# EspressoSystems/cap

Hardware: AMD Instinct MI355X
Metric: transfer-note proofs/sec (2-in/2-out) (higher is better)
Workload: dtype u32 limbs (254-bit Montgomery integers; 9 x 29-bit lazy limbs in the hot kernels)

## Files before the change

cap_amd/csrc/curve29.hpp:

```cpp
#pragma once
#include "curve.hpp"
#include "field29.hpp"

namespace cap {

struct g1a {
  fl x, y;
};
struct g1x {
  fl x, y, zz, zzz;
};

template <int SCHED>
struct G1LT {
  using F = Fl<FqP29, SCHED>;

  static CAP_HD bool all_zero(const fl& a) {
    uint32_t o = 0;
#pragma unroll
    for (int i = 0; i < 9; i++) o |= a.v[i];
    return o == 0;
  }
  static CAP_HD bool is_inf(const g1x& p) { return all_zero(p.zz); }
  static CAP_HD bool is_inf(const g1a& p) { return all_zero(p.x) && all_zero(p.y); }
// ... 116 lines not shown
    const fl p = F::sub(u2, a.x);
    if (F::is_zero(p)) return false;
#if defined(__HIP_DEVICE_COMPILE__)
    asm volatile("; madd_acc: common path");
#endif
    const fl r = F::sub(s2, a.y);
    const fl pp = F::sqr(p);
    const fl ppp = F::mul(p, pp);
    const fl qq = F::mul(a.x, pp);
    g1x o;
    o.x = F::weak_reduce(F::sub_from_lazy(F::sub2p_lazy(F::sqr(r), ppp), F::add(qq, qq)));
    o.y = F::mul_add_mul(r, F::sub2p_lazy(qq, o.x), F::neg4p_lazy(a.y), ppp);
    o.zz = F::mul(a.zz, pp);
    o.zzz = F::mul(a.zzz, ppp);
    a = o;
    return true;
  }
  static CAP_HD bool add_acc(g1x& a, const g1x& b) {
    const fl u1 = F::mul(a.x, b.zz);
    const fl u2 = F::mul(b.x, a.zz);
    const fl p = F::sub(u2, u1);
    if (F::is_zero(p)) return false;
    const fl s1 = F::mul(a.y, b.zzz);
    const fl s2 = F::mul(b.y, a.zzz);
    const fl r = F::sub(s2, s1);
    const fl pp = F::sqr(p);
    const fl ppp = F::mul(p, pp);
    const fl qq = F::mul(u1, pp);
    g1x o;
    o.x = F::weak_reduce(F::sub_from_lazy(F::sub2p_lazy(F::sqr(r), ppp), F::add(qq, qq)));
// ... 102 lines not shown
```

cap_amd/csrc/msm.hip:

```cpp
#define CAP_FL_SCHED 1
#include "msm.hpp"
#include "msm_recode.hpp"
#include "curve29.hpp"
#include "quad29.hpp"
#include "launch.hpp"

#include <math.h>
#include <stdio.h>

#include <atomic>
#include <stdlib.h>

namespace cap {

namespace {

constexpr int kThreads = 256;
constexpr uint32_t kDigitTile = 1024;
constexpr int kDigitThreads = 1024;
constexpr uint32_t kMinItemLen = 32, kMaxItemLen = 512;
constexpr uint32_t kBatchItemCap = 256;

using G1S = G1LT<0>;

// ... 894 lines not shown
      if ((uint64_t)chunk * blockDim.x >= n_items) break;
      it = chunk * blockDim.x + threadIdx.x;
    } else {
      it = (blockIdx.x + round * gridDim.x) * blockDim.x + threadIdx.x;
      if ((uint64_t)(blockIdx.x + round * gridDim.x) * blockDim.x >= n_items) break;
    }
    if (it >= n_items) continue;
  const uint32_t gb = item_bucket[it], j = item_sub[it];
  const uint32_t b = gb / half;
  const uint32_t cnt = counts[gb];
  const uint32_t items = (cnt + item_len - 1) / item_len;
  const uint32_t q = cnt / items, r = cnt - q * items;
  const uint32_t lo = j * q + (j < r ? j : r), hi = lo + q + (j < r ? 1u : 0u);
  const uint32_t* lst = sorted + (size_t)b * per + offsets[gb];
  g1x acc = G1L::inf();
  for (uint32_t e = lo; e < hi; e++) {
    const uint32_t v = lst[e];
    const g1a pt = G1L::load(ext[v & 0x7FFFFFFFu]);
    const bool negate = (v >> 31) != 0;
    if (__builtin_expect(G1L::is_inf(pt) || !G1L::madd_acc(acc, pt, negate), 0)) acc = G1L::add_mixed(acc, pt, negate);
  }
  if (items == 1) buckets[gb] = G1L::store(acc);
  else item_pts[item_base[b] + item_off[gb] + j] = G1L::store(acc);
  }
}

__global__ __launch_bounds__(kThreads) void msm_reduce_segments(const g1_xyzz* __restrict__ buckets, uint32_t half,
                                                                uint32_t seg_len, uint32_t nseg, uint32_t batch,
                                                                g1_xyzz* __restrict__ seg_pts) {
  uint32_t t = blockIdx.x * blockDim.x + threadIdx.x;
  if (t >= nseg * batch) return;
// ... 1701 lines not shown
```

cap_amd/csrc/ntt.hip:

```cpp
#include "ntt.hpp"
#include "field29.hpp"
#include "launch.hpp"

#include <stdlib.h>

#include <vector>

namespace cap {

namespace {

constexpr int kThreads = 256;
#ifndef CAP_NTT_IO_BATCH
#define CAP_NTT_IO_BATCH 2
#endif
constexpr int kIoBatch = CAP_NTT_IO_BATCH;
#ifdef CAP_NTT_WAVES4
#define CAP_NTT_ATTR __attribute__((amdgpu_waves_per_eu(4, 4)))
#else
#define CAP_NTT_ATTR
#endif
constexpr uint32_t kMaxTileLogDefault = 10;
uint32_t max_tile_log() {
  static uint32_t v = [] {
// ... 22 lines not shown
  uint32_t in_group;
  uint32_t in_es;
  size_t in_inner2;
  uint32_t in_group2;
  size_t out_outer, out_inner;
  uint32_t out_group;
  size_t out_inner2;
  uint32_t out_group2;
  size_t pre_inner;
  const fl* tw_small;
  const fe* tw_full;
  const fe* pre_scale;
  const fe* post_scale;
  fe post_scalar;
  uint32_t use_post_scalar;
  uint32_t lazy_out;
  uint32_t log_n;
  uint32_t log_len;
  uint32_t log_c;
  uint32_t log_m;
  uint32_t log_n1, log_n2;
  uint32_t* tile_counter;
  uint32_t tiles_x, tiles_y;
};

__device__ __forceinline__ bool next_tile(const PassParams& p, uint32_t round, uint32_t& bx, uint32_t& by) {
  if (!p.tile_counter) {
    bx = blockIdx.x;
    by = blockIdx.y;
    return round == 0;
// ... 152 lines not shown
      if (p.pre_scale && any[u] && nz) v = Fr29::mul(v, Fr29::load(pre[u]));
      sh[(bitrev32(j, p.log_len) << p.log_c) + c] = v;
    }
  }
  __syncthreads();
  lds_ntt(sh, p.tw_small, p.log_len, p.log_c);
  const uint32_t tw_shift = p.log_n - p.log_m;
  for (uint32_t e0 = threadIdx.x; e0 < tile; e0 += kIoBatch * kThreads) {
    fe tw[kIoBatch];
    size_t exs[kIoBatch];
#pragma unroll
    for (int u = 0; u < kIoBatch; u++) {
      const uint32_t e = e0 + u * kThreads;
      const uint32_t c = e & cmask, k = e >> p.log_c;
      exs[u] = e < tile ? ((size_t)(col0 + c) * k) << tw_shift : 0;
      if (exs[u]) tw[u] = p.tw_full[exs[u]];
    }
#pragma unroll
    for (int u = 0; u < kIoBatch; u++) {
      const uint32_t e = e0 + u * kThreads;
      if (e >= tile) break;
      const uint32_t c = e & cmask, k = e >> p.log_c;
      fl v = sh[e];
      v = exs[u] ? Fr29::mul(v, Fr29::load(tw[u])) : Fr29::weak_reduce(v);
      out[base + ((size_t)k << log_s) + c] = Fr29::pack(v);
    }
  }
  }
}
template <bool PERSIST>
__global__ __launch_bounds__(kThreads) CAP_NTT_ATTR void ntt_col_pass(PassParams p) {
  extern __shared__ __align__(16) unsigned char smem[];
  fl* sh = reinterpret_cast<fl*>(smem);
  if constexpr (!PERSIST) {
    col_tile(p, sh, blockIdx.x, blockIdx.y);
  } else {
    uint32_t bx, by;
    for (uint32_t round = 0; next_tile(p, round, bx, by); round++) col_tile(p, sh, bx, by);
  }
// ... 235 lines not shown
  hipError_t e;
  if ((e = hipMalloc(&d->tw_fwd, sizeof(fe) * n)) != hipSuccess) return (int)e;
  if ((e = hipMalloc(&d->tw_inv, sizeof(fe) * n)) != hipSuccess) return (int)e;
  if ((e = hipMalloc(&d->coset_fwd, sizeof(fe) * n)) != hipSuccess) return (int)e;
  if ((e = hipMalloc(&d->coset_inv, sizeof(fe) * n)) != hipSuccess) return (int)e;
  fe w = host_root_of_unity(log_n);
  fe g = host_from_u64(5);
  d->n_inv = Fr::inv(host_from_u64((uint64_t)n));
  int rc;
  if ((rc = build_powers(d->tw_fwd, n, w, nullptr, stream))) return rc;
  if ((rc = build_powers(d->tw_inv, n, Fr::inv(w), nullptr, stream))) return rc;
  if ((rc = build_powers(d->coset_fwd, n, g, nullptr, stream))) return rc;
  if ((rc = build_powers(d->coset_inv, n, Fr::inv(g), &d->n_inv, stream))) return rc;
  fe* src[4] = {d->tw_fwd, d->tw_inv, d->coset_fwd, d->coset_inv};
  fe** dst[4] = {&d->tw29_fwd, &d->tw29_inv, &d->coset29_fwd, &d->coset29_inv};
  for (int k = 0; k < 4; k++) {
    if ((e = hipMalloc(dst[k], sizeof(fe) * n)) != hipSuccess) return (int)e;
    launch("table_to_internal", table_to_internal, dim3((unsigned)((n + 255) / 256)), dim3(256), 0, stream, *dst[k],
           (const fe*)src[k], n);
  }
  d->n_inv29 = Fr29::pack(Fr29::canonical(Fr29::from_ext(d->n_inv)));
  if ((e = hipStreamSynchronize(stream)) != hipSuccess) return (int)e;
  hipFree(d->tw_inv);
  hipFree(d->coset_fwd);
  hipFree(d->coset_inv);
  d->tw_inv = d->coset_fwd = d->coset_inv = nullptr;
  return 0;
}

void ntt_free_domain(NttDomain* d) {
  if (d->tw_fwd) hipFree(d->tw_fwd);
  if (d->tw_inv) hipFree(d->tw_inv);
  if (d->coset_fwd) hipFree(d->coset_fwd);
  if (d->coset_inv) hipFree(d->coset_inv);
  for (fe* t : {d->tw29_fwd, d->tw29_inv, d->coset29_fwd, d->coset29_inv})
    if (t) hipFree(t);
  d->tw_fwd = d->tw_inv = d->coset_fwd = d->coset_inv = nullptr;
  d->tw29_fwd = d->tw29_inv = d->coset29_fwd = d->coset29_inv = nullptr;
}

void ntt_table_to_internal(fe* out, const fe* in, size_t n, hipStream_t stream) {
  if (n == 0) return;
  launch("table_to_internal", table_to_internal, dim3((unsigned)((n + 255) / 256)), dim3(256), 0, stream, out, in, n);
}

namespace {
unsigned ntt_persistent() {
  static const unsigned v = [] {
    const char* e = getenv("CAPGPU_NTT_PERSISTENT");
    const long x = e ? atol(e) : 0;
    return (unsigned)(x >= 1 && x <= 16 ? x : 0);
  }();
  return v;
// ... 116 lines not shown
  auto set_out = [&](const Addr& a) {
    p.out_outer = a.outer;
    p.out_inner = a.inner;
    p.out_group = a.group;
    p.out_group2 = 1;
    p.out_inner2 = 0;
    if (&a == &a_dst && io && io->dst_group2 > 1) {
      p.out_group2 = io->dst_group2;
      p.out_inner2 = io->dst_inner2;
    }
  };
  p.pre_inner = io ? io->pre_inner : 0;
  p.log_n = log_n;
  p.tw_full = tw_full;
  p.use_post_scalar = 0;

  const fe* pre = (!dir && coset) ? dom.coset29_fwd : nullptr;
  if (io && io->pre_scale) pre = io->pre_scale;
  bool first = true;
  const fe* cur_in = io ? io->src : data;
  uint32_t log_m = log_n;
  for (int d = 0; d < passes - 1; d++) {
    const uint32_t log_len = plan.digits[d], log_c = plan.log_c[d];
    p.in = cur_in;
    p.out = scratch;
    set_in(first ? a_src : a_tmp, first ? src_len : ~(size_t)0, first ? src_es : 1);
    set_out(a_tmp);
    p.tw_small = reinterpret_cast<const fl*>(tws[log_len]);
    p.pre_scale = first ? pre : nullptr;
    p.post_scale = nullptr;
    p.log_len = log_len;
    p.log_c = log_c;
    p.log_m = log_m;
    size_t lds = sizeof(fl) << (log_len + log_c);
    launch_pass("ntt_col_pass", ntt_col_pass<false>, ntt_col_pass<true>, p, small, (size_t)plan.tiles[d], count, lds,
                plan.persistent[d] != 0, stream);
    cur_in = scratch;
    first = false;
    log_m -= log_len;
  }
  {
    const int last = passes - 1;
    const uint32_t log_len = plan.digits[last], log_c = plan.log_c[last];
    const uint32_t log_n1 = passes >= 2 ? plan.digits[0] : 0;
    const uint32_t log_n2 = passes == 3 ? plan.digits[1] : 0;
    p.in = cur_in;
    p.out = data;
    set_in(first ? a_src : a_tmp, first ? src_len : ~(size_t)0, first ? src_es : 1);
    set_out(a_dst);
    p.tw_small = reinterpret_cast<const fl*>(tws[log_len]);
    p.pre_scale = first ? pre : nullptr;
    p.post_scale = (dir && coset) ? dom.coset29_inv : nullptr;
    p.use_post_scalar = (dir && !coset) ? 1 : 0;
    p.post_scalar = (io && io->has_post_scalar) ? io->post_scalar : dom.n_inv29;
    p.lazy_out = (io && io->lazy_out) ? 1 : 0;
    p.log_len = log_len;
    p.log_c = log_c;
    p.log_n1 = log_n1;
    p.log_n2 = log_n2;
    size_t lds = sizeof(fl) << (log_len + log_c);
    launch_pass("ntt_row_pass", ntt_row_pass<false>, ntt_row_pass<true>, p, small, (size_t)plan.tiles[last], count, lds,
                plan.persistent[last] != 0, stream);
  }
  return 0;
}

namespace {
void exponent_third(uint32_t e[8]) {
// ... 114 lines not shown
```

cap_amd/csrc/ntt.hpp:

```cpp
#pragma once
#include <hip/hip_runtime.h>
#include <stdint.h>

#include "field.hpp"

namespace cap {

struct NttDomain {
  uint32_t log_n = 0;
  fe* tw_fwd = nullptr;
  fe* tw_inv = nullptr;
  fe* coset_fwd = nullptr;
  fe* coset_inv = nullptr;
  fe n_inv;
  fe* tw29_fwd = nullptr;
  fe* tw29_inv = nullptr;
  fe* coset29_fwd = nullptr;
  fe* coset29_inv = nullptr;
  fe n_inv29;
};

constexpr int kMaxLogTile = 11;
struct NttSmallTables {
  fe* fwd[kMaxLogTile + 1] = {nullptr};
  fe* inv[kMaxLogTile + 1] = {nullptr};
  uint32_t* fwd_u[kMaxLogTile + 1] = {nullptr};
  uint32_t* inv_u[kMaxLogTile + 1] = {nullptr};
  uint32_t* pass_counters = nullptr;
  mutable uint32_t next_counter = 0;
};
constexpr uint32_t kNttPassCounters = 256;
// ... 61 lines not shown
```

cap_amd/csrc/plonk.hip:

```cpp
#define CAP_FL_SCHED 1
#include <stdlib.h>
#include <string.h>

#include <algorithm>
#include <atomic>
#include <chrono>
#include <condition_variable>
#include <functional>
#include <map>
#include <mutex>
#include <string>
#include <thread>
#include <vector>

#include "check_kernels.hpp"
#include "coalescer.hpp"
#include "context.hpp"
#include "host_util.hpp"
#include "launch.hpp"
#include "params.hpp"
#include "plonk_kernels.hpp"
#include "tickets.hpp"
#include "transcript_dev.hpp"
#include "vars_kernels.hpp"
// ... 529 lines not shown
      x = Fr::mul(x, w6);
    }
  }
  const Ntt3Domain* dom_m = nullptr;
  if ((rc = get_domain3(K.log_m, &dom_m))) return rc;
  launch("k_inv_nx1", k_inv_nx1, dim3(cdiv(m, kThreads)), dim3(kThreads), 0, s, K.inv_nx1, (const fe*)dom_m->xs_ext,
         fr_from_u64((uint64_t)n), m);
  ntt_table_to_internal(K.inv_nx1, K.inv_nx1, m, s);
  {
    auto conv = [](const fe& a) { return Fr29::pack(Fr29::canonical(Fr29::from_ext(a))); };
    K.qc29.g = conv(K.qc.g);
    for (int i = 0; i < NW; i++) K.qc29.k[i] = conv(K.qc.k[i]);
    for (int i = 0; i < 8; i++) K.qc29.zh_inv[i] = conv(K.qc.zh_inv[i]);
  }
  if (!K.recompute) {
    CAP_HIP(hipMalloc(&K.pk_coset, sizeof(fe) * 18 * m));
    if ((rc = compute_pk_coset(s, K, K.pk_coset))) return rc;
  }
  return CAPGPU_OK;
}

void key_set_vk(ProvingKey& K, const std::vector<g1_affine>& ha) {
  memset(&K.vk, 0, sizeof(K.vk));
  K.vk.domain_size = K.n;
  K.vk.num_inputs = K.num_inputs;
  for (int i = 0; i < NW; i++) fe_to_words(K.qc.k[i], K.vk.k[i]);
  for (int i = 0; i < NS; i++) affine_to_words(ha[i], K.vk.selector_comms[i]);
  for (int i = 0; i < NW; i++) affine_to_words(ha[NS + i], K.vk.sigma_comms[i]);
  SolidityTranscript t;
  t.append_u64_le(254);
  t.append_u64_le((uint64_t)K.n);
  t.append_u64_le((uint64_t)K.num_inputs);
// ... 147 lines not shown
  K->qc = src.qc;
  K->qc29 = src.qc29;
  K->vk = src.vk;
  K->vk_bytes = src.vk_bytes;
  K->recompute = src.recompute;
  K->device = c.device;
  auto dup = [&](fe** dst, const fe* from, size_t count) -> int {
    if (!from) return CAPGPU_OK;
    CAP_HIP(hipMalloc(dst, sizeof(fe) * count));
    CAP_HIP(copy_between(*dst, c.device, from, src_device, sizeof(fe) * count, c.stream));
    return CAPGPU_OK;
  };
  int rc;
  if ((rc = dup(&K->coef, src.coef, 18 * src.ps))) return rc;
  if ((rc = dup(&K->sig_eval, src.sig_eval, (size_t)NW * src.n))) return rc;
  if ((rc = dup(&K->pk_coset, src.pk_coset, 18 * src.m))) return rc;
  if ((rc = dup(&K->inv_nx1, src.inv_nx1, src.m))) return rc;
  {
    std::lock_guard<std::mutex> lk(src.chk_mu);
    if (src.wire_vars && src.chk_perm) {
      const size_t bytes = sizeof(uint32_t) * NW * src.n;
      CAP_HIP(hipMalloc(&K->wire_vars, bytes));
      CAP_HIP(hipMalloc(&K->chk_perm, bytes));
      CAP_HIP(copy_between(K->wire_vars, c.device, src.wire_vars, src_device, bytes, c.stream));
      CAP_HIP(copy_between(K->chk_perm, c.device, src.chk_perm, src_device, bytes, c.stream));
      K->num_vars = src.num_vars;
    }
  }
  CAP_HIP(hipStreamSynchronize(c.stream));
  *out = K;
  return CAPGPU_OK;
// ... 1729 lines not shown
```

cap_amd/csrc/plonk_kernels.hpp:

```cpp
#pragma once
#include <hip/hip_runtime.h>

#include "field.hpp"
#include "field29.hpp"

namespace cap {
namespace pk {

constexpr int NW = 5;
constexpr int NS = 13;
constexpr int kThreads = 256;
constexpr int kScanPerThread = 4;
constexpr int kScanBlock = kThreads * kScanPerThread;

struct Chal {
  fe beta, gamma, alpha, alpha2;
};

struct QuotConst {
  fe g;
  fe k[NW];
  fe zh_inv[8];
};

__global__ __launch_bounds__(kThreads) void k_pad_copy(fe* __restrict__ dst, size_t dst_outer, size_t dst_inner,
                                                       const fe* __restrict__ src, size_t src_outer, size_t src_inner,
                                                       uint32_t inner, size_t len, size_t total) {
  size_t k = (size_t)blockIdx.x * blockDim.x + threadIdx.x;
  if (k >= total) return;
  uint32_t q = blockIdx.y;
  size_t d = (size_t)(q / inner) * dst_outer + (size_t)(q % inner) * dst_inner + k;
// ... 185 lines not shown
struct ColAcc {
  uint64_t c[18];
  __device__ __forceinline__ void clear() {
#pragma unroll
    for (int k = 0; k < 18; k++) c[k] = 0;
  }
  __device__ __forceinline__ void mad(const fl& a, const fl& b) {
#pragma unroll
    for (int i = 0; i < 9; i++)
#pragma unroll
      for (int j = 0; j < 9; j++) c[i + j] += (uint64_t)a.v[i] * b.v[j];
  }
  __device__ __forceinline__ fl reduce() { return Fr29::reduce_cols(c); }
};

__global__ __launch_bounds__(kThreads) void k_quotient(const fe* __restrict__ pkc, const fe* const* __restrict__ pkc_of,
                                                       const fe* __restrict__ cos, const fe* __restrict__ xs,
                                                       const fe* __restrict__ inv_nx1,
                                                       const Chal* __restrict__ chal, QuotConst qc, size_t m,
                                                       fe* __restrict__ t_out) {
  using F = Fr29;
  size_t i = (size_t)blockIdx.y * blockDim.x + threadIdx.x;
  if (i >= m) return;
  const uint32_t p = blockIdx.x;
  if (pkc_of) pkc = pkc_of[p];
  const uint32_t mm = (uint32_t)(m / 3);
  const uint32_t blk = (i >= mm ? 1u : 0u) + (i >= 2 * (size_t)mm ? 1u : 0u);
  const fe* c = cos + (size_t)p * 6 * m;
  auto sel = [&](int s) { return F::load(pkc[(size_t)s * m + i]); };
  fl w0 = F::load(c[i]), w1 = F::load(c[m + i]), w2 = F::load(c[2 * m + i]), w3 = F::load(c[3 * m + i]),
     w4 = F::load(c[4 * m + i]);
  fl w01 = F::mul(w0, w1), w23 = F::mul(w2, w3);
  ColAcc acc;
  acc.clear();
  acc.mad(sel(0), w0);
  acc.mad(sel(1), w1);
  acc.mad(sel(2), w2);
  acc.mad(sel(3), w3);
  acc.mad(sel(4), w01);
// ... 2 lines not shown
  acc.clear();
  {
    fl t = F::sqr(w0);
    acc.mad(sel(6), F::mul(F::sqr(t), w0));
    t = F::sqr(w1);
    acc.mad(sel(7), F::mul(F::sqr(t), w1));
    t = F::sqr(w2);
    acc.mad(sel(8), F::mul(F::sqr(t), w2));
    t = F::sqr(w3);
    acc.mad(sel(9), F::mul(F::sqr(t), w3));
  }
  acc.mad(sel(12), F::mul(F::mul(w01, w23), w4));
  acc.mad(F::neg(sel(10)), w4);
  fl gate2 = acc.reduce();
  fl total = F::normalize(F::add(F::add(gate, gate2), sel(11)));
  const fl beta = F::load(chal[p].beta), gamma = F::load(chal[p].gamma);
  const fl zx = F::load(c[5 * m + i]);
  {
    fl x = F::load(xs[i]);
    fl bx = F::mul(beta, x);
    const uint32_t k1 = (uint32_t)i - blk * mm;
    const size_t inext = (size_t)blk * mm + ((k1 + 2) & (mm - 1));
    fl a = zx, b = F::load(c[5 * m + inext]);
    fl wg = F::add(w0, gamma);
    a = F::mul(a, F::normalize(F::add(wg, bx)));
    b = F::mul(b, F::normalize(F::add(wg, F::mul(beta, sel(NS + 0)))));
    wg = F::add(w1, gamma);
    a = F::mul(a, F::normalize(F::add(wg, F::mul(F::load(qc.k[1]), bx))));
    b = F::mul(b, F::normalize(F::add(wg, F::mul(beta, sel(NS + 1)))));
    wg = F::add(w2, gamma);
    a = F::mul(a, F::normalize(F::add(wg, F::mul(F::load(qc.k[2]), bx))));
    b = F::mul(b, F::normalize(F::add(wg, F::mul(beta, sel(NS + 2)))));
    wg = F::add(w3, gamma);
    a = F::mul(a, F::normalize(F::add(wg, F::mul(F::load(qc.k[3]), bx))));
    b = F::mul(b, F::normalize(F::add(wg, F::mul(beta, sel(NS + 3)))));
    wg = F::add(w4, gamma);
    a = F::mul(a, F::normalize(F::add(wg, F::mul(F::load(qc.k[4]), bx))));
// ... 150 lines not shown
```

cap_amd/csrc/prove_run.hpp:

```cpp
#pragma once
#include "context.hpp"
#include "host_util.hpp"
#include "launch.hpp"
#include "params.hpp"
#include "plonk_kernels.hpp"
#include "transcript_dev.hpp"
#include "vars_kernels.hpp"

namespace cap {
namespace {

inline unsigned cdiv(size_t a, size_t b) { return (unsigned)((a + b - 1) / b); }

void pad_copy(hipStream_t s, fe* dst, size_t dst_outer, size_t dst_inner, const fe* src, size_t src_outer,
              size_t src_inner, uint32_t inner, uint32_t count, size_t len, size_t total) {
  if (count == 0 || total == 0) return;
  launch("k_pad_copy", k_pad_copy, dim3(cdiv(total, kThreads), count), dim3(kThreads), 0, s, dst, dst_outer, dst_inner,
         src, src_outer, src_inner, inner, len, total);
}

template <int OP, int REV>
void scan_exclusive(hipStream_t s, const fe* in, fe* out, size_t len, size_t stride, uint32_t batch, fe* tot) {
  uint32_t nblocks = cdiv(len, kScanBlock);
  launch(OP == 0 ? "k_scan_local_mul" : "k_scan_local_add", k_scan_local<OP, REV>, dim3(nblocks, batch), dim3(kThreads),
// ... 133 lines not shown
BatchWs carve(void* base, const ProvingKey& K, uint32_t P, size_t num_inputs, bool coeffs, uint32_t tr_stride = 0) {
  Carver c(base);
  BatchWs w{};
  size_t n = K.n, m = K.m, ps = K.ps;
  w.wpoly = c.take<fe>((size_t)P * NW * ps);
  w.wev = coeffs ? c.take<fe>((size_t)P * NW * n) : nullptr;
  w.pi = num_inputs ? c.take<fe>((size_t)P * n) : nullptr;
  w.num = c.take<fe>((size_t)P * n);
  w.den = c.take<fe>((size_t)P * n);
  w.pre = c.take<fe>((size_t)P * n);
  w.sfx = c.take<fe>((size_t)P * n);
  w.scan_tot = c.take<fe>((size_t)P * 2 * (cdiv(ps, kScanBlock) + 1));
  w.inv_total = c.take<fe>(P);
  w.zpoly = c.take<fe>((size_t)P * ps);
  w.coset = c.take<fe>((size_t)P * 6 * m);
  w.pkc = K.recompute ? c.take<fe>((size_t)18 * m) : nullptr;
  w.t = c.take<fe>((size_t)P * m);
  w.pows = c.take<fe>((size_t)P * 4 * ps);
  w.pw = c.take<fe>((size_t)P * 4 * 24);
  w.pows_small = c.take<fe>((size_t)P * 4 * (kPowLow + (ps + kPowLow - 1) / kPowLow));
  w.batchpoly = c.take<fe>((size_t)P * 2 * ps);
  w.hbuf = c.take<fe>((size_t)P * 2 * ps);
  w.quot = c.take<fe>((size_t)P * 2 * ps);
  w.evals = c.take<fe>((size_t)P * 10);
  w.eval_partial = c.take<fe>((size_t)P * 10 * kEvalChunks);
  w.d_pub = c.take<fe>((size_t)P * (num_inputs ? num_inputs : 1));
  w.d_blind = c.take<fe>((size_t)P * 13);
  w.chal = c.take<Chal>(P);
  w.chal29 = c.take<Chal>(P);
  w.flags = c.take<uint32_t>(P);
  w.comms = c.take<g1_jac>((size_t)P * 5);
// ... 3 lines not shown
  if (tr_stride) {
    w.d_proofs = c.take<uint8_t>((size_t)P * td::kPrBytes);
    w.zeta = c.take<fe>(P);
    w.tr_state = c.take<uint8_t>((size_t)P * 64);
    w.tr_app = c.take<uint8_t>((size_t)P * td::kAppBytes);
    w.tr_pre_len = c.take<uint32_t>(P);
    w.tr_pre = c.take<uint8_t>((size_t)P * tr_stride);
  }
  w.total = c.off + 256;
  return w;
}

int compute_pk_coset(hipStream_t s, const ProvingKey& K, fe* dst) {
  return run_ntt3_fwd(s, K.log_m, dst, 18, NttIo{K.coef, K.ps, 0, K.n, 1, K.m, 0, 1});
}

std::atomic<int> g_wire_commit{-1};
bool wire_commit_from_evals() {
  static const int env_default = [] {
    const char* e = getenv("CAPGPU_WIRE_COMMIT");
    return (e && (!strcmp(e, "coeffs") || !strcmp(e, "0"))) ? 0 : 1;
  }();
  const int m = g_wire_commit.load(std::memory_order_relaxed);
  return (m < 0 ? env_default : m) != 0;
}

std::atomic<int> g_transcript{-1};
int transcript_mode() {
  static const int env_default = [] {
    const char* e = getenv("CAPGPU_TRANSCRIPT");
// ... 160 lines not shown
    if (!sizing) trace("pb_lagrange_fallback", c.slot, rc);
  }
  pl.dev_tr = transcript_mode() == CAPGPU_TRANSCRIPT_DEVICE && !comm_shard_prover();
  if (pl.dev_tr) {
    if (longest_prefix > (1u << 30)) {
      set_error("capgpu_plonk_prove: transcript init message of %zu bytes", longest_prefix);
      return CAPGPU_ERR_INVALID_ARG;
    }
    pl.tr_stride = transcript_stride(longest_prefix);
  }
  pl.inv_on_device = perm_inv_on_device() || pl.dev_tr;
  pl.chunks = pl.r1_copies ? h2d_chunks(P) : 1;
  const bool own = !c.prof.on && c.stream == c.own_stream;
  pl.overlap = pl.chunks == 1 && P <= r1_overlap_max() && (sizing || (own && !comm_shard_prover())) &&
               (pl.s2 = side_stream(c)) != nullptr;
  pl.graphs = P <= graph_max_batch() && pl.chunks == 1 && own && comm_shard_slot() < 0;
  *out = pl;
  return CAPGPU_OK;
}

struct ProveNeeds {
  size_t prove_ws = 0, msm_ws = 0, ntt_scratch = 0, stage_a = 0, stage_b = 0, pinned = 0;
  void ntt(size_t bytes) { ntt_scratch = std::max(ntt_scratch, bytes); }
  void msm(const MsmBases& T, size_t len, uint32_t batch) { msm_ws = std::max(msm_ws, msm_workspace_bytes(T, len, batch)); }
};

struct ProveRequest {
  const fe* d_wires = nullptr;
  const uint64_t* pub_inputs = nullptr;
  size_t num_inputs = 0;
  const uint64_t* blinders = nullptr;
// ... 26 lines not shown
  const uint32_t P;
  const size_t n, m, ps, num_inputs;
  const fe* const d_wires;
  const uint64_t* pub_inputs;
  const uint64_t* const* h_wires;
  const NttDomain* dom_n = nullptr;
  const Ntt3Domain* dom_q = nullptr;
  const fe omega;
  std::vector<uint64_t> pub_rows;
  std::vector<const fe*> key_ptrs;
  const fe* const* sig_of = nullptr;
  const fe* const* pkc_of = nullptr;
  std::vector<SolidityTranscript> tr;
  g1_jac* hj = nullptr;
  fe* h_tot = nullptr;
  fe* h_evals = nullptr;
  uint32_t* h_flags = nullptr;
  uint8_t* h_proofs = nullptr;
  const size_t proofs_bytes;
  std::vector<g1_affine> ha;

  ProveRun(Context& c_, const ProvePlan& pl_, const ProvingKey& K_, const ProveRequest& rq_)
      : side_drain{c_, false}, c(c_), s(c_.stream), pl(pl_), K(K_), rq(rq_), P(pl_.P), n(K_.n), m(K_.m), ps(K_.ps),
        num_inputs(rq_.num_inputs), d_wires(rq_.d_wires), pub_inputs(rq_.pub_inputs),
        h_wires(pl_.r1_copies ? rq_.h_wires : nullptr), omega(ntt_root_of_unity(K_.log_n)),
        proofs_bytes((size_t)pl_.P * td::kPrBytes) {}
  ProveRun(const ProveRun&) = delete;
  ProveRun& operator=(const ProveRun&) = delete;

  const ProvingKey& key_of(uint32_t p) const { return rq.keys ? *(*rq.keys)[p] : K; }
// ... 312 lines not shown
             (const fe*)w.den, n, w.inv_total, P);
    } else {
      launch("k_perm_total", k_perm_total, dim3(cdiv(P, 64)), dim3(64), 0, s, (const fe*)w.sfx, (const fe*)w.den, n,
             w.inv_total, P);
      return CAPGPU_OK;
    }
    return finish_and_commit_z();
  }

  int r3_body() {
    int r;
    const fe* pkc = K.pk_coset;
    if (K.recompute) {
      for (uint32_t p = 0; p < P; p++)
        if ((r = compute_pk_coset(s, K, w.pkc))) return r;
      pkc = w.pkc;
    }
    launch("k_quotient", k_quotient, dim3(P, cdiv(m, kThreads)), dim3(kThreads), 0, s, pkc, pkc_of,
           (const fe*)w.coset, (const fe*)dom_q->xs29, (const fe*)K.inv_nx1, (const Chal*)w.chal29, K.qc29, m, w.t);
    if ((r = run_ntt3_inv(s, K.log_m, w.t, P, w.pi))) return r;
    {
      size_t lo = NW * (n + 1) + 3;
      launch("k_check_degree", k_check_degree, dim3(cdiv(m - (lo - 1), kThreads), P), dim3(kThreads), 0, s,
             (const fe*)w.t, m, lo, w.flags);
    }
    return run_msm(s, *pl.B, w.t, m, NW, n + 2, n + 2, P * NW, w.comms);
  }
  static void r3_needs(const ProvePlan& pl, const ProvingKey& K, uint32_t cnt, ProveNeeds& nd) {
    if (K.recompute) nd.ntt(ntt3_scratch(K.log_m, 18));
    nd.ntt(ntt3_scratch(K.log_m, cnt));
    nd.msm(*pl.B, K.n + 2, cnt * NW);
  }

  std::vector<EvalDesc> make_edesc() const {
// ... 136 lines not shown
           return seg(1, [&]() -> int { return r3_wire_cosets(s); });
         })))
      return rc;
    trace("pb_r1_done", c.slot);
    std::vector<Chal> chal(P);
    parallel_for(P, [&](uint32_t p) {
      for (int i = 0; i < NW; i++) {
        append_g1(tr[p], ha[p * NW + i]);
        affine_to_words(ha[p * NW + i], proofs[p].wires_poly_comms[i]);
      }
      (void)get_challenge(tr[p]);
      chal[p].beta = get_challenge(tr[p]);
      chal[p].gamma = get_challenge(tr[p]);
      chal[p].alpha = Fr::zero();
      chal[p].alpha2 = Fr::zero();
    });
    CAP_HIP(hipMemcpyAsync(w.chal, chal.data(), sizeof(Chal) * P, hipMemcpyHostToDevice, s));

    if ((rc = seg(2, [&]() -> int { return r2_body(); }))) return rc;
    if (!pl.inv_on_device) {
      std::vector<fe> pref(P);
      fe* tot = h_tot;
      CAP_HIP(hipMemcpyAsync(tot, w.inv_total, sizeof(fe) * P, hipMemcpyDeviceToHost, s));
      CAP_HIP(wait_stream());
      fe acc = Fr::one();
      for (uint32_t p = 0; p < P; p++) {
        pref[p] = acc;
        if (!Fr::is_zero(tot[p])) acc = Fr::mul(acc, tot[p]);
      }
      acc = Fr::inv_fermat(acc);
      for (uint32_t p = P; p-- > 0;) {
// ... 4 lines not shown
      }
      CAP_HIP(hipMemcpyAsync(w.inv_total, tot, sizeof(fe) * P, hipMemcpyHostToDevice, s));
      if ((rc = seg(7, [&]() -> int { return finish_and_commit_z(); }))) return rc;
    }
    if ((rc = fetch_comms(P, [&]() -> int {
           if (pl.overlap) return CAPGPU_OK;
           return seg(3, [&]() -> int { return z_cosets(s); });
         })))
      return rc;
    trace("pb_r2_done", c.slot);
    parallel_for(P, [&](uint32_t p) {
      append_g1(tr[p], ha[p]);
      affine_to_words(ha[p], proofs[p].prod_perm_poly_comm);
      chal[p].alpha = get_challenge(tr[p]);
      chal[p].alpha2 = Fr::sqr(chal[p].alpha);
    });
    CAP_HIP(hipMemcpyAsync(w.chal, chal.data(), sizeof(Chal) * P, hipMemcpyHostToDevice, s));
    std::vector<Chal> chal29(P);
    parallel_for(P, [&](uint32_t p) {
      auto conv = [](const fe& a) { return Fr29::pack(Fr29::canonical(Fr29::from_ext(a))); };
      chal29[p].beta = conv(chal[p].beta);
      chal29[p].gamma = conv(chal[p].gamma);
      chal29[p].alpha = conv(chal[p].alpha);
      chal29[p].alpha2 = conv(chal[p].alpha2);
    });
    CAP_HIP(hipMemcpyAsync(w.chal29, chal29.data(), sizeof(Chal) * P, hipMemcpyHostToDevice, s));

    if ((rc = seg(4, [&]() -> int { return r3_body(); }))) return rc;
    uint32_t* flags = h_flags;
    CAP_HIP(hipMemcpyAsync(flags, w.flags, sizeof(uint32_t) * P, hipMemcpyDeviceToHost, s));
    if ((rc = fetch_comms(P * NW))) return rc;
    trace("pb_r3_done", c.slot);
    if ((rc = degree_verdict(flags))) return rc;
    std::vector<fe> zeta(P);
    std::vector<fe> pw((size_t)P * 4 * 24);
    parallel_for(P, [&](uint32_t p) {
      for (int i = 0; i < NW; i++) {
        append_g1(tr[p], ha[p * NW + i]);
        affine_to_words(ha[p * NW + i], proofs[p].split_quot_poly_comms[i]);
// ... 62 lines not shown
```

cap_amd/csrc/transcript_dev.hpp:

```cpp
#pragma once
#include <stddef.h>
#include <stdint.h>

#include "curve.hpp"
#include "field29.hpp"
#if defined(__HIPCC__) && !defined(CAP_TD_NO_KERNELS)
#include "plonk_kernels.hpp"
#endif

namespace cap {
namespace td {

struct SpongeMsg {
  const uint8_t *a, *b, *c;
  uint32_t la, lb, lc;
  uint32_t fork;
};
constexpr uint32_t kRate = 136;
CAP_HD uint32_t sponge_len(const SpongeMsg& m) { return m.la + m.lb + m.lc + m.fork; }
CAP_HD uint32_t sponge_blocks(const SpongeMsg& m) { return sponge_len(m) / kRate + 1; }
CAP_HD uint8_t sponge_byte(const SpongeMsg& m, uint32_t len, uint32_t end, uint32_t k, uint32_t half) {
  uint8_t v = 0;
  if (k < m.la) v = m.a[k];
  else if (k < m.la + m.lb) v = m.b[k - m.la];
// ... 361 lines not shown
      compress_g1(out[i], t.app + (size_t)p * kAppBytes + app_off + 32 * i);
    }
  }
  __syncthreads();
  KeccakTabs<LaneDev> tabs;
  tabs.init();
  constexpr uint32_t lapp = app_off + 32 * NPTS;
  if (ROUND == 1) {
    (void)draw(t, p, lapp, tabs);
    const fe beta = draw(t, p, lapp, tabs), gamma = draw(t, p, lapp, tabs);
    if (threadIdx.x == 0) {
      chal[p].beta = beta;
      chal[p].gamma = gamma;
      chal[p].alpha = Fr::zero();
      chal[p].alpha2 = Fr::zero();
      chal29[p].beta = to_internal(beta);
      chal29[p].gamma = to_internal(gamma);
      chal29[p].alpha = Fr::zero();
      chal29[p].alpha2 = Fr::zero();
    }
  } else if (ROUND == 2) {
    const fe alpha = draw(t, p, lapp, tabs);
    if (threadIdx.x == 0) {
      const fe a2 = Fr::sqr(alpha);
      chal[p].alpha = alpha;
      chal[p].alpha2 = a2;
      chal29[p].alpha = to_internal(alpha);
      chal29[p].alpha2 = to_internal(a2);
    }
  } else {
    const fe zeta = draw(t, p, lapp, tabs);
    if (threadIdx.x == 0) {
      zeta_out[p] = zeta;
      fe b4[4];
      zeta_bases(zeta, omega, b4);
      for (int q = 0; q < 4; q++) sh[q] = b4[q];
    }
    __syncthreads();
    if (threadIdx.x < 4) {
      fe x = sh[threadIdx.x];
      for (int b = 0; b < 24; b++) {
        pw[((size_t)p * 4 + threadIdx.x) * 24 + b] = x;
        x = Fr::sqr(x);
// ... 52 lines not shown
```

Baseline: 1406.

## Fold beta into permutation quotient, n^-1 into inverse NTT twiddles, pair-add MSM buckets

Bundles three unrelated optimizations. The quotient kernel now divides the permutation terms by beta, using precomputed k_j*x columns and an alpha*beta^5 factor, which removes per-element beta*x multiplies and normalizations at the cost of extra pk_coset columns and a second pass when beta may be zero. The inverse NTT's first pass now uses a twiddle table pre-scaled by n^-1, which removes the separate post-scalar multiply. MSM bucket accumulation now starts with an affine+affine pair add to skip the first mixed-add multiplies. CUDA graphs are disabled unless the fold mode is the default.

```diff
diff --git a/cap_amd/csrc/curve29.hpp b/cap_amd/csrc/curve29.hpp
--- a/cap_amd/csrc/curve29.hpp
+++ b/cap_amd/csrc/curve29.hpp
@@ -154,6 +154,24 @@
     o.zz = F::mul(a.zz, pp);
     o.zzz = F::mul(a.zzz, ppp);
     a = o;
+    return true;
+  }
+  static CAP_HD bool add_affine_pair(g1x& out, const g1a& q0, bool neg0, const g1a& q1, bool neg1) {
+    const fl p = F::sub2p(q1.x, q0.x);
+    if (F::is_zero(p)) return false;
+    const fl n0 = F::neg2p_lazy(q0.y);
+    const fl y0 = neg0 ? n0 : q0.y, my0 = neg0 ? q0.y : n0;
+    const fl y1 = neg1 ? F::neg2p_lazy(q1.y) : q1.y;
+    const fl r = F::sub(y1, y0);
+    const fl pp = F::sqr(p);
+    const fl ppp = F::mul(p, pp);
+    const fl qq = F::mul(q0.x, pp);
+    g1x o;
+    o.x = F::weak_reduce(F::sub_from_lazy(F::sub2p_lazy(F::sqr(r), ppp), F::add(qq, qq)));
+    o.y = F::mul_add_mul(r, F::sub2p_lazy(qq, o.x), my0, ppp);
+    o.zz = pp;
+    o.zzz = ppp;
+    out = o;
     return true;
   }
   static CAP_HD bool add_acc(g1x& a, const g1x& b) {
diff --git a/cap_amd/csrc/msm.hip b/cap_amd/csrc/msm.hip
--- a/cap_amd/csrc/msm.hip
+++ b/cap_amd/csrc/msm.hip
@@ -932,7 +932,16 @@
   const uint32_t lo = j * q + (j < r ? j : r), hi = lo + q + (j < r ? 1u : 0u);
   const uint32_t* lst = sorted + (size_t)b * per + offsets[gb];
   g1x acc = G1L::inf();
-  for (uint32_t e = lo; e < hi; e++) {
+  uint32_t e = lo;
+#ifndef CAP_ACC_NO_PAIR
+  if (hi - lo >= 2) {
+    const uint32_t v0 = lst[lo], v1 = lst[lo + 1];
+    const g1a p0 = G1L::load(ext[v0 & 0x7FFFFFFFu]), p1 = G1L::load(ext[v1 & 0x7FFFFFFFu]);
+    if (!G1L::is_inf(p0) && !G1L::is_inf(p1) && G1L::add_affine_pair(acc, p0, (v0 >> 31) != 0, p1, (v1 >> 31) != 0))
+      e = lo + 2;
+  }
+#endif
+  for (; e < hi; e++) {
     const uint32_t v = lst[e];
     const g1a pt = G1L::load(ext[v & 0x7FFFFFFFu]);
     const bool negate = (v >> 31) != 0;
diff --git a/cap_amd/csrc/ntt.hip b/cap_amd/csrc/ntt.hip
--- a/cap_amd/csrc/ntt.hip
+++ b/cap_amd/csrc/ntt.hip
@@ -60,6 +60,7 @@
   const fe* post_scale;
   fe post_scalar;
   uint32_t use_post_scalar;
+  uint32_t tw_scaled;
   uint32_t lazy_out;
   uint32_t log_n;
   uint32_t log_len;
@@ -242,7 +243,7 @@
       const uint32_t e = e0 + u * kThreads;
       const uint32_t c = e & cmask, k = e >> p.log_c;
       exs[u] = e < tile ? ((size_t)(col0 + c) * k) << tw_shift : 0;
-      if (exs[u]) tw[u] = p.tw_full[exs[u]];
+      if (exs[u] || p.tw_scaled) tw[u] = p.tw_full[exs[u]];
     }
 #pragma unroll
     for (int u = 0; u < kIoBatch; u++) {
@@ -250,7 +251,7 @@
       if (e >= tile) break;
       const uint32_t c = e & cmask, k = e >> p.log_c;
       fl v = sh[e];
-      v = exs[u] ? Fr29::mul(v, Fr29::load(tw[u])) : Fr29::weak_reduce(v);
+      v = (exs[u] || p.tw_scaled) ? Fr29::mul(v, Fr29::load(tw[u])) : Fr29::weak_reduce(v);
       out[base + ((size_t)k << log_s) + c] = Fr29::pack(v);
     }
   }
@@ -516,6 +517,12 @@
   if ((rc = build_powers(d->coset_inv, n, Fr::inv(g), &d->n_inv, stream))) return rc;
   fe* src[4] = {d->tw_fwd, d->tw_inv, d->coset_fwd, d->coset_inv};
   fe** dst[4] = {&d->tw29_fwd, &d->tw29_inv, &d->coset29_fwd, &d->coset29_inv};
+#ifndef CAP_NTT_NO_INV_FOLD
+  if ((e = hipMalloc(&d->tw29_inv_n, sizeof(fe) * n)) != hipSuccess) return (int)e;
+  if ((rc = build_powers(d->tw29_inv_n, n, Fr::inv(w), &d->n_inv, stream))) return rc;
+  launch("table_to_internal", table_to_internal, dim3((unsigned)((n + 255) / 256)), dim3(256), 0, stream, d->tw29_inv_n,
+         (const fe*)d->tw29_inv_n, n);
+#endif
   for (int k = 0; k < 4; k++) {
     if ((e = hipMalloc(dst[k], sizeof(fe) * n)) != hipSuccess) return (int)e;
     launch("table_to_internal", table_to_internal, dim3((unsigned)((n + 255) / 256)), dim3(256), 0, stream, *dst[k],
@@ -535,10 +542,10 @@
   if (d->tw_inv) hipFree(d->tw_inv);
   if (d->coset_fwd) hipFree(d->coset_fwd);
   if (d->coset_inv) hipFree(d->coset_inv);
-  for (fe* t : {d->tw29_fwd, d->tw29_inv, d->coset29_fwd, d->coset29_inv})
+  for (fe* t : {d->tw29_fwd, d->tw29_inv, d->tw29_inv_n, d->coset29_fwd, d->coset29_inv})
     if (t) hipFree(t);
   d->tw_fwd = d->tw_inv = d->coset_fwd = d->coset_inv = nullptr;
-  d->tw29_fwd = d->tw29_inv = d->coset29_fwd = d->coset29_inv = nullptr;
+  d->tw29_fwd = d->tw29_inv = d->tw29_inv_n = d->coset29_fwd = d->coset29_inv = nullptr;
 }
 
 void ntt_table_to_internal(fe* out, const fe* in, size_t n, hipStream_t stream) {
@@ -685,6 +692,11 @@
   p.log_n = log_n;
   p.tw_full = tw_full;
   p.use_post_scalar = 0;
+#ifndef CAP_NTT_NO_INV_FOLD
+  const bool inv_fold = dir && !coset && passes >= 2 && !(io && io->has_post_scalar) && dom.tw29_inv_n;
+#else
+  const bool inv_fold = false;
+#endif
 
   const fe* pre = (!dir && coset) ? dom.coset29_fwd : nullptr;
   if (io && io->pre_scale) pre = io->pre_scale;
@@ -703,6 +715,8 @@
     p.log_len = log_len;
     p.log_c = log_c;
     p.log_m = log_m;
+    p.tw_full = (inv_fold && d == 0) ? dom.tw29_inv_n : tw_full;
+    p.tw_scaled = (inv_fold && d == 0) ? 1 : 0;
     size_t lds = sizeof(fl) << (log_len + log_c);
     launch_pass("ntt_col_pass", ntt_col_pass<false>, ntt_col_pass<true>, p, small, (size_t)plan.tiles[d], count, lds,
                 plan.persistent[d] != 0, stream);
@@ -722,7 +736,7 @@
     p.tw_small = reinterpret_cast<const fl*>(tws[log_len]);
     p.pre_scale = first ? pre : nullptr;
     p.post_scale = (dir && coset) ? dom.coset29_inv : nullptr;
-    p.use_post_scalar = (dir && !coset) ? 1 : 0;
+    p.use_post_scalar = (dir && !coset && !inv_fold) ? 1 : 0;
     p.post_scalar = (io && io->has_post_scalar) ? io->post_scalar : dom.n_inv29;
     p.lazy_out = (io && io->lazy_out) ? 1 : 0;
     p.log_len = log_len;
diff --git a/cap_amd/csrc/ntt.hpp b/cap_amd/csrc/ntt.hpp
--- a/cap_amd/csrc/ntt.hpp
+++ b/cap_amd/csrc/ntt.hpp
@@ -15,6 +15,7 @@
   fe n_inv;
   fe* tw29_fwd = nullptr;
   fe* tw29_inv = nullptr;
+  fe* tw29_inv_n = nullptr;
   fe* coset29_fwd = nullptr;
   fe* coset29_inv = nullptr;
   fe n_inv29;
diff --git a/cap_amd/csrc/plonk.hip b/cap_amd/csrc/plonk.hip
--- a/cap_amd/csrc/plonk.hip
+++ b/cap_amd/csrc/plonk.hip
@@ -567,8 +567,9 @@
     for (int i = 0; i < 8; i++) K.qc29.zh_inv[i] = conv(K.qc.zh_inv[i]);
   }
   if (!K.recompute) {
-    CAP_HIP(hipMalloc(&K.pk_coset, sizeof(fe) * 18 * m));
+    CAP_HIP(hipMalloc(&K.pk_coset, sizeof(fe) * kPkcCols * m));
     if ((rc = compute_pk_coset(s, K, K.pk_coset))) return rc;
+    if ((rc = compute_pk_kx(s, K, K.pk_coset))) return rc;
   }
   return CAPGPU_OK;
 }
@@ -746,7 +747,7 @@
   int rc;
   if ((rc = dup(&K->coef, src.coef, 18 * src.ps))) return rc;
   if ((rc = dup(&K->sig_eval, src.sig_eval, (size_t)NW * src.n))) return rc;
-  if ((rc = dup(&K->pk_coset, src.pk_coset, 18 * src.m))) return rc;
+  if ((rc = dup(&K->pk_coset, src.pk_coset, kPkcCols * src.m))) return rc;
   if ((rc = dup(&K->inv_nx1, src.inv_nx1, src.m))) return rc;
   {
     std::lock_guard<std::mutex> lk(src.chk_mu);
diff --git a/cap_amd/csrc/plonk_kernels.hpp b/cap_amd/csrc/plonk_kernels.hpp
--- a/cap_amd/csrc/plonk_kernels.hpp
+++ b/cap_amd/csrc/plonk_kernels.hpp
@@ -9,12 +9,14 @@
 
 constexpr int NW = 5;
 constexpr int NS = 13;
+constexpr int NKX = NW - 1;
+constexpr int kPkcCols = NS + NW + NKX;
 constexpr int kThreads = 256;
 constexpr int kScanPerThread = 4;
 constexpr int kScanBlock = kThreads * kScanPerThread;
 
 struct Chal {
-  fe beta, gamma, alpha, alpha2;
+  fe beta, gamma, alpha, alpha2, beta_inv, alpha_beta5;
 };
 
 struct QuotConst {
@@ -230,15 +232,33 @@
   __device__ __forceinline__ fl reduce() { return Fr29::reduce_cols(c); }
 };
 
+__global__ __launch_bounds__(kThreads) void k_kx_columns(fe* __restrict__ dst, const fe* __restrict__ xs, QuotConst qc,
+                                                         size_t m) {
+  using F = Fr29;
+  size_t i = (size_t)blockIdx.x * blockDim.x + threadIdx.x;
+  if (i >= m) return;
+  const fl x = F::load(xs[i]);
+#pragma unroll
+  for (int j = 0; j < NKX; j++) dst[(size_t)j * m + i] = F::pack(F::canonical(F::mul(F::load(qc.k[j + 1]), x)));
+}
+
+__device__ __forceinline__ bool fe_nonzero(const fe& a) {
+  uint32_t o = 0;
+#pragma unroll
+  for (int k = 0; k < 8; k++) o |= a.v[k];
+  return o != 0;
+}
+template <bool FOLD>
 __global__ __launch_bounds__(kThreads) void k_quotient(const fe* __restrict__ pkc, const fe* const* __restrict__ pkc_of,
                                                        const fe* __restrict__ cos, const fe* __restrict__ xs,
                                                        const fe* __restrict__ inv_nx1,
                                                        const Chal* __restrict__ chal, QuotConst qc, size_t m,
-                                                       fe* __restrict__ t_out) {
+                                                       uint32_t only_unfoldable, fe* __restrict__ t_out) {
   using F = Fr29;
   size_t i = (size_t)blockIdx.y * blockDim.x + threadIdx.x;
   if (i >= m) return;
   const uint32_t p = blockIdx.x;
+  if (FOLD ? !fe_nonzero(chal[p].beta_inv) : (only_unfoldable && fe_nonzero(chal[p].beta_inv))) return;
   if (pkc_of) pkc = pkc_of[p];
   const uint32_t mm = (uint32_t)(m / 3);
   const uint32_t blk = (i >= mm ? 1u : 0u) + (i >= 2 * (size_t)mm ? 1u : 0u);
@@ -271,13 +291,33 @@
   acc.mad(F::neg(sel(10)), w4);
   fl gate2 = acc.reduce();
   fl total = F::normalize(F::add(F::add(gate, gate2), sel(11)));
-  const fl beta = F::load(chal[p].beta), gamma = F::load(chal[p].gamma);
+  const fl gamma = F::load(chal[p].gamma);
   const fl zx = F::load(c[5 * m + i]);
-  {
+  const uint32_t k1 = (uint32_t)i - blk * mm;
+  const size_t inext = (size_t)blk * mm + ((k1 + 2) & (mm - 1));
+  if constexpr (FOLD) {
+    const fl beta_inv = F::load(chal[p].beta_inv);
+    fl a = zx, b = F::load(c[5 * m + inext]);
+    fl u = F::mul(F::add(w0, gamma), beta_inv);
+    a = F::mul(a, F::add(u, F::load(xs[i])));
+    b = F::mul(b, F::add(u, sel(NS + 0)));
+    u = F::mul(F::add(w1, gamma), beta_inv);
+    a = F::mul(a, F::add(u, sel(NS + NW + 0)));
+    b = F::mul(b, F::add(u, sel(NS + 1)));
+    u = F::mul(F::add(w2, gamma), beta_inv);
+    a = F::mul(a, F::add(u, sel(NS + NW + 1)));
+    b = F::mul(b, F::add(u, sel(NS + 2)));
+    u = F::mul(F::add(w3, gamma), beta_inv);
+    a = F::mul(a, F::add(u, sel(NS + NW + 2)));
+    b = F::mul(b, F::add(u, sel(NS + 3)));
+    u = F::mul(F::add(w4, gamma), beta_inv);
+    a = F::mul(a, F::add(u, sel(NS + NW + 3)));
+    b = F::mul(b, F::add(u, sel(NS + 4)));
+    total = F::normalize(F::add(total, F::mul(F::load(chal[p].alpha_beta5), F::sub(a, b))));
+  } else {
+    const fl beta = F::load(chal[p].beta);
     fl x = F::load(xs[i]);
     fl bx = F::mul(beta, x);
-    const uint32_t k1 = (uint32_t)i - blk * mm;
-    const size_t inext = (size_t)blk * mm + ((k1 + 2) & (mm - 1));
     fl a = zx, b = F::load(c[5 * m + inext]);
     fl wg = F::add(w0, gamma);
     a = F::mul(a, F::normalize(F::add(wg, bx)));
diff --git a/cap_amd/csrc/prove_run.hpp b/cap_amd/csrc/prove_run.hpp
--- a/cap_amd/csrc/prove_run.hpp
+++ b/cap_amd/csrc/prove_run.hpp
@@ -171,7 +171,7 @@
   w.inv_total = c.take<fe>(P);
   w.zpoly = c.take<fe>((size_t)P * ps);
   w.coset = c.take<fe>((size_t)P * 6 * m);
-  w.pkc = K.recompute ? c.take<fe>((size_t)18 * m) : nullptr;
+  w.pkc = K.recompute ? c.take<fe>((size_t)kPkcCols * m) : nullptr;
   w.t = c.take<fe>((size_t)P * m);
   w.pows = c.take<fe>((size_t)P * 4 * ps);
   w.pw = c.take<fe>((size_t)P * 4 * 24);
@@ -205,6 +205,18 @@
 int compute_pk_coset(hipStream_t s, const ProvingKey& K, fe* dst) {
   return run_ntt3_fwd(s, K.log_m, dst, 18, NttIo{K.coef, K.ps, 0, K.n, 1, K.m, 0, 1});
 }
+int compute_pk_kx(hipStream_t s, const ProvingKey& K, fe* dst) {
+  const Ntt3Domain* dq = nullptr;
+  if (int rc = get_domain3(K.log_m, &dq)) return rc;
+  launch("k_kx_columns", k_kx_columns, dim3(cdiv(K.m, kThreads)), dim3(kThreads), 0, s, dst + (size_t)18 * K.m,
+         (const fe*)dq->xs29, K.qc29, K.m);
+  return CAPGPU_OK;
+}
+int quotient_fold() {
+  const char* e = getenv("CAPGPU_QUOT_FOLD");
+  const int v = e ? atoi(e) : 1;
+  return v >= 0 && v <= 2 ? v : 1;
+}
 
 std::atomic<int> g_wire_commit{-1};
 bool wire_commit_from_evals() {
@@ -395,7 +407,7 @@
   const bool own = !c.prof.on && c.stream == c.own_stream;
   pl.overlap = pl.chunks == 1 && P <= r1_overlap_max() && (sizing || (own && !comm_shard_prover())) &&
                (pl.s2 = side_stream(c)) != nullptr;
-  pl.graphs = P <= graph_max_batch() && pl.chunks == 1 && own && comm_shard_slot() < 0;
+  pl.graphs = P <= graph_max_batch() && pl.chunks == 1 && own && comm_shard_slot() < 0 && quotient_fold() == 1;
   *out = pl;
   return CAPGPU_OK;
 }
@@ -452,6 +464,7 @@
   std::vector<SolidityTranscript> tr;
   g1_jac* hj = nullptr;
   fe* h_tot = nullptr;
+  bool beta_zero_possible = true;
   fe* h_evals = nullptr;
   uint32_t* h_flags = nullptr;
   uint8_t* h_proofs = nullptr;
@@ -794,10 +807,19 @@
     if (K.recompute) {
       for (uint32_t p = 0; p < P; p++)
         if ((r = compute_pk_coset(s, K, w.pkc))) return r;
+      if ((r = compute_pk_kx(s, K, w.pkc))) return r;
       pkc = w.pkc;
     }
-    launch("k_quotient", k_quotient, dim3(P, cdiv(m, kThreads)), dim3(kThreads), 0, s, pkc, pkc_of,
-           (const fe*)w.coset, (const fe*)dom_q->xs29, (const fe*)K.inv_nx1, (const Chal*)w.chal29, K.qc29, m, w.t);
+    const int fold = quotient_fold();
+    if (fold == 2)
+      CAP_HIP(hipMemset2DAsync(&w.chal29[0].beta_inv, sizeof(Chal), 0, sizeof(fe), P, s));
+    if (fold)
+      launch("k_quotient", k_quotient<true>, dim3(P, cdiv(m, kThreads)), dim3(kThreads), 0, s, pkc, pkc_of,
+             (const fe*)w.coset, (const fe*)dom_q->xs29, (const fe*)K.inv_nx1, (const Chal*)w.chal29, K.qc29, m, 1u, w.t);
+    if (!fold || fold == 2 || beta_zero_possible)
+      launch("k_quotient_direct", k_quotient<false>, dim3(P, cdiv(m, kThreads)), dim3(kThreads), 0, s,
+             pkc, pkc_of, (const fe*)w.coset, (const fe*)dom_q->xs29, (const fe*)K.inv_nx1, (const Chal*)w.chal29, K.qc29, m,
+             fold ? 1u : 0u, w.t);
     if ((r = run_ntt3_inv(s, K.log_m, w.t, P, w.pi))) return r;
     {
       size_t lo = NW * (n + 1) + 3;
@@ -964,7 +986,11 @@
       chal[p].gamma = get_challenge(tr[p]);
       chal[p].alpha = Fr::zero();
       chal[p].alpha2 = Fr::zero();
+      chal[p].beta_inv = Fr::is_zero(chal[p].beta) ? Fr::zero() : Fr::inv(chal[p].beta);
+      chal[p].alpha_beta5 = Fr::zero();
     });
+    beta_zero_possible = pl.graphs;
+    for (uint32_t p = 0; p < P; p++) beta_zero_possible = beta_zero_possible || Fr::is_zero(chal[p].beta);
     CAP_HIP(hipMemcpyAsync(w.chal, chal.data(), sizeof(Chal) * P, hipMemcpyHostToDevice, s));
 
     if ((rc = seg(2, [&]() -> int { return r2_body(); }))) return rc;
@@ -999,6 +1025,8 @@
       affine_to_words(ha[p], proofs[p].prod_perm_poly_comm);
       chal[p].alpha = get_challenge(tr[p]);
       chal[p].alpha2 = Fr::sqr(chal[p].alpha);
+      const fe b2 = Fr::sqr(chal[p].beta);
+      chal[p].alpha_beta5 = Fr::mul(chal[p].alpha, Fr::mul(Fr::sqr(b2), chal[p].beta));
     });
     CAP_HIP(hipMemcpyAsync(w.chal, chal.data(), sizeof(Chal) * P, hipMemcpyHostToDevice, s));
     std::vector<Chal> chal29(P);
@@ -1008,6 +1036,8 @@
       chal29[p].gamma = conv(chal[p].gamma);
       chal29[p].alpha = conv(chal[p].alpha);
       chal29[p].alpha2 = conv(chal[p].alpha2);
+      chal29[p].beta_inv = conv(chal[p].beta_inv);
+      chal29[p].alpha_beta5 = conv(chal[p].alpha_beta5);
     });
     CAP_HIP(hipMemcpyAsync(w.chal29, chal29.data(), sizeof(Chal) * P, hipMemcpyHostToDevice, s));
 
diff --git a/cap_amd/csrc/transcript_dev.hpp b/cap_amd/csrc/transcript_dev.hpp
--- a/cap_amd/csrc/transcript_dev.hpp
+++ b/cap_amd/csrc/transcript_dev.hpp
@@ -399,10 +399,15 @@
       chal[p].gamma = gamma;
       chal[p].alpha = Fr::zero();
       chal[p].alpha2 = Fr::zero();
+      const fe beta_inv = fr_inv_public(beta);
+      chal[p].beta_inv = beta_inv;
+      chal[p].alpha_beta5 = Fr::zero();
       chal29[p].beta = to_internal(beta);
       chal29[p].gamma = to_internal(gamma);
       chal29[p].alpha = Fr::zero();
       chal29[p].alpha2 = Fr::zero();
+      chal29[p].beta_inv = to_internal(beta_inv);
+      chal29[p].alpha_beta5 = Fr::zero();
     }
   } else if (ROUND == 2) {
     const fe alpha = draw(t, p, lapp, tabs);
@@ -412,6 +417,10 @@
       chal[p].alpha2 = a2;
       chal29[p].alpha = to_internal(alpha);
       chal29[p].alpha2 = to_internal(a2);
+      const fe beta = chal[p].beta, b2 = Fr::sqr(beta);
+      const fe ab5 = Fr::mul(alpha, Fr::mul(Fr::sqr(b2), beta));
+      chal[p].alpha_beta5 = ab5;
+      chal29[p].alpha_beta5 = to_internal(ab5);
     }
   } else {
     const fe zeta = draw(t, p, lapp, tabs);
```

New measurement: 1436 (median of 6 runs). 1.02x the previous value.
